# Veason-silverbullet/DIGAT

Measured on NVIDIA B200. Metric: impressions_scored_per_sec, higher is better.
Workload: dtype f32

## Files before the change

digat_b200/csrc/pair_attention_sparse.cuh:

```cuda
#pragma once
#include "common.cuh"
#include "tma.cuh"
#include "pair_attention.cuh"

namespace digat {

#ifndef DIGAT_SPARSE_WARPS
#define DIGAT_SPARSE_WARPS 10
#endif
#ifndef DIGAT_SPARSE_BUFS
#define DIGAT_SPARSE_BUFS 4
#endif
#ifndef DIGAT_SPARSE_MINCTAS
#define DIGAT_SPARSE_MINCTAS 2
#endif
#ifndef DIGAT_SPARSE_UNROLL
#define DIGAT_SPARSE_UNROLL 4
#endif
constexpr int kSparseConsumers = 32 * DIGAT_SPARSE_WARPS;
constexpr int kSparseThreads = kSparseConsumers + 32;
constexpr int kSparseBufs = DIGAT_SPARSE_BUFS;
constexpr int kSparseDc1 = 32, kSparseDc3 = 64;
constexpr int kSparseUnroll = DIGAT_SPARSE_UNROLL;

struct SparseGeom {
    int nch1, nch3;
    int G;
    int stagger_lo, stagger_hi;
    int tile_floats;
    int unit_floats;
    size_t smem;
};

__device__ __forceinline__ void consumer_sync() {
    asm volatile("bar.sync 1, %0;" :: "n"(kSparseConsumers) : "memory");
}

template <bool kIndexed, bool kMulti, bool kTrain = false>
__global__ void __launch_bounds__(kSparseThreads, DIGAT_SPARSE_MINCTAS)
graph_layer_fwd_sparse_kernel(const __grid_constant__ CUtensorMap map1, const __grid_constant__ CUtensorMap map3,
                              PairAttnArgs p, SparseGeom g) {
    extern __shared__ __align__(1024) uint8_t smem_raw[];
    const int tid = threadIdx.x, lane = tid & 31, warp = tid >> 5;
    const int n = p.n, D = p.D;
    const int b = kMulti ? blockIdx.x * g.G : blockIdx.x;
    const int N = kMulti ? min(g.G, p.B - b) * n : n;
    const int NB = kMulti ? g.G * n : n;
    const int src0 = kIndexed ? p.px_index[b] : b;

    float* ring = reinterpret_cast<float*>(smem_raw);
    uint64_t* full = reinterpret_cast<uint64_t*>(ring + kSparseBufs * g.unit_floats);
    uint64_t* empty = full + kSparseBufs;
    float* a_s = reinterpret_cast<float*>(empty + kSparseBufs);
    float* k3_s = a_s + D;
    float* score = k3_s + D;
    int* rowptr = reinterpret_cast<int*>(score + NB * n);
    uint16_t* meta = reinterpret_cast<uint16_t*>(rowptr + (NB + 2));
    uint8_t* adj_s = reinterpret_cast<uint8_t*>((reinterpret_cast<uintptr_t>(meta + NB * n) + 15) & ~(uintptr_t)15);
    uint8_t* uniform_row = adj_s + ((NB * n + 15) & ~15);
    uint8_t* dead_row = uniform_row + NB;
    int* pos_s = reinterpret_cast<int*>((reinterpret_cast<uintptr_t>(dead_row + NB) + 3) & ~(uintptr_t)3);
    int* n_act_s = pos_s + NB;
    uint8_t* act_list = reinterpret_cast<uint8_t*>(n_act_s + 1);

    if (tid == 0) {
        for (int i = 0; i < kSparseBufs; ++i) {
            mbar_init(&full[i], 1);
            mbar_init(&empty[i], kSparseConsumers / 32);
        }
        asm volatile("fence.mbarrier_init.release.cluster;" ::: "memory");
    }
#ifdef DIGAT_SPARSE_STAGGER
    if (blockIdx.x >= gridDim.y * 0 + (unsigned)g.stagger_lo && blockIdx.x < (unsigned)g.stagger_hi) __nanosleep(DIGAT_SPARSE_STAGGER);
#endif
    __syncthreads();
    const int n_loads = g.nch1 + g.nch3;

    if (warp == kSparseConsumers / 32) {
        if (lane == 0) {
            for (int l = 0; l < n_loads; ++l) {
                const int buf = l % kSparseBufs;
                float* dst = ring + buf * g.unit_floats;
                mbar_wait(&empty[buf], ((uint32_t)(l / kSparseBufs) & 1u) ^ 1u);
                if (l < g.nch1) {
                    mbar_arrive_expect_tx(&full[buf], 2u * NB * kSparseDc1 * 4u);
                    tma_load_2d(dst, &map1, &full[buf], D + l * kSparseDc1, src0 * n);
                    tma_load_2d(dst + g.tile_floats, &map1, &full[buf], 2 * D + l * kSparseDc1, src0 * n);
                } else {
                    mbar_arrive_expect_tx(&full[buf], (uint32_t)NB * kSparseDc3 * 4u);
                    tma_load_2d(dst, &map3, &full[buf], (l - g.nch1) * kSparseDc3, src0 * n);
                }
            }
        }
        return;
    }

#ifdef DIGAT_TC_TIMING
    const long long t0 = clock64();
    long long ta = t0, wait1 = 0, wait3 = 0;
#endif
    const float* __restrict__ gat_s = p.gat_s;
    for (int i = tid; i < D / 4; i += kSparseConsumers) {
        if (gat_s == nullptr) reinterpret_cast<float4*>(a_s)[i] = reinterpret_cast<const float4*>(p.a)[i];
        if (kIndexed) reinterpret_cast<float4*>(k3_s)[i] = reinterpret_cast<const float4*>(p.k3 + (size_t)b * p.ldk3)[i];
    }
    const bool have_csr = !kMulti && p.csr_rowptr != nullptr;
    if (have_csr) {
        const size_t cg = p.csr_index != nullptr ? (size_t)p.csr_index[b] : (size_t)b;
        const uint16_t* rp = p.csr_rowptr + cg * (n + 1);
        for (int i = tid; i <= n; i += kSparseConsumers) {
            const uint32_t raw = rp[i];
            rowptr[i] = (int)(raw & 0x7fffu);
            if (i > 0) uniform_row[i - 1] = (uint8_t)(raw >> 15);
        }
        if (p.Yc != nullptr)
            for (int i = tid; i < N; i += kSparseConsumers) pos_s[i] = p.row_pos[(size_t)b * n + i];
        consumer_sync();
        const int Ec = rowptr[n];
        const uint16_t* mg = p.csr_meta + cg * (size_t)n * n;
        for (int e = tid; e < Ec; e += kSparseConsumers) {
            const uint32_t mt = mg[e];
            meta[e] = (uint16_t)mt;
            score[e] = gat_s == nullptr ? 0.f
                                        : gat_s[((size_t)b * n + (mt & 255u)) * 2] + gat_s[((size_t)b * n + (mt >> 8)) * 2 + 1];
        }
        for (int i = tid; i < N; i += kSparseConsumers) dead_row[i] = rowptr[i + 1] == rowptr[i];
        if (warp == 0) {
            int run_a = 0;
            for (int base = 0; base < N; base += 32) {
                const int i = base + lane;
                const bool alive = i < N && rowptr[i + 1] != rowptr[i];
                const unsigned m = __ballot_sync(0xffffffffu, alive);
                if (alive) act_list[run_a + __popc(m & ((1u << lane) - 1u))] = (uint8_t)i;
                run_a += __popc(m);
            }
            if (lane == 0) *n_act_s = run_a;
        }
    } else {
    {
        const uint8_t* adj_g = p.adj + (p.adj_index != nullptr ? (size_t)p.adj_index[b] : (size_t)b) * n * n;
        const int n2 = N * n;
        if (((n2 | (int)(reinterpret_cast<uintptr_t>(adj_g) & 15)) & 15) == 0) {
            for (int i = tid; i < n2 / 16; i += kSparseConsumers)
                reinterpret_cast<uint4*>(adj_s)[i] = __ldg(reinterpret_cast<const uint4*>(adj_g) + i);
        } else {
            for (int i = tid; i < n2; i += kSparseConsumers) adj_s[i] = adj_g[i];
        }
        for (int i = tid; i < N; i += kSparseConsumers) {
            dead_row[i] = (p.row_active != nullptr && p.row_active[(size_t)b * n + i] == 0) ? 1 : 0;
            if (p.Yc != nullptr) pos_s[i] = p.row_pos[(size_t)b * n + i];
        }
    }
    consumer_sync();
#ifdef DIGAT_TC_TIMING
    ta = clock64();
#endif
    for (int i = warp; i < N; i += kSparseConsumers / 32) {
        const bool dead = dead_row[i] != 0;
        int deg = 0;
        if (!dead)
            for (int k = 0; k < (n + 31) / 32; ++k) {
                const int j = lane + 32 * k;
                deg += __popc(__ballot_sync(0xffffffffu, j < n && adj_s[i * n + j] != 0));
            }
        if (lane == 0) {
            uniform_row[i] = deg == 0 && !dead;
            rowptr[i + 1] = dead ? 0 : (deg == 0 ? n : deg);
        }
    }
    consumer_sync();
    if (warp == 0) {
        int run_e = 0;
        for (int base = 0; base < N; base += 32) {
            const int i = base + lane;
            int ve = i < N ? rowptr[i + 1] : 0;
#pragma unroll
            for (int o = 1; o < 32; o <<= 1) {
                const int te = __shfl_up_sync(0xffffffffu, ve, o);
                if (lane >= o) ve += te;
            }
            if (i < N) rowptr[i + 1] = run_e + ve;
            run_e += __shfl_sync(0xffffffffu, ve, 31);
        }
        if (lane == 0) rowptr[0] = 0;
        int run_a = 0;
        for (int base = 0; base < N; base += 32) {
            const int i = base + lane;
            const bool alive = i < N && dead_row[i] == 0;
            const unsigned m = __ballot_sync(0xffffffffu, alive);
            if (alive) act_list[run_a + __popc(m & ((1u << lane) - 1u))] = (uint8_t)i;
            run_a += __popc(m);
        }
        if (lane == 0) *n_act_s = run_a;
    }
    consumer_sync();
    for (int i = warp; i < N; i += kSparseConsumers / 32) {
        const int e0 = rowptr[i];
        const bool uni = uniform_row[i] != 0;
        if (dead_row[i] != 0) continue;
        const int node0 = kMulti ? (i / n) * n : 0;
        int filled = 0;
        for (int k = 0; k < (n + 31) / 32; ++k) {
            const int j = lane + 32 * k;
            const bool on = j < n && (uni || adj_s[i * n + j] != 0);
            const unsigned m = __ballot_sync(0xffffffffu, on);
            if (on) {
                const int e = e0 + filled + __popc(m & ((1u << lane) - 1u));
                meta[e] = (uint16_t)((node0 + j) | (i << 8));
                score[e] = gat_s == nullptr ? 0.f
                                            : gat_s[((size_t)b * n + node0 + j) * 2] + gat_s[((size_t)b * n + i) * 2 + 1];
            }
            filled += __popc(m);
        }
    }
    }
    const int E = rowptr[N];
    consumer_sync();

#ifdef DIGAT_TC_TIMING
    const long long t1 = clock64();
#endif
    const uint32_t a_off = (uint32_t)(reinterpret_cast<uint8_t*>(a_s) - smem_raw);
    const uint32_t k3_off = (uint32_t)(reinterpret_cast<uint8_t*>(k3_s) - smem_raw);
    for (int l = 0; l < g.nch1; ++l) {
        const int buf = l % kSparseBufs;
        const int c0 = l * kSparseDc1;
        const int wq = min(kSparseDc1, D - c0) >> 2;
        const uint32_t uoff = (uint32_t)(buf * g.unit_floats) * 4u;
        const uint32_t koff = uoff + (uint32_t)g.tile_floats * 4u;
        const uint32_t aoff = a_off + (uint32_t)c0 * 4u, k3off = k3_off + (uint32_t)c0 * 4u;
#ifdef DIGAT_TC_TIMING
        const long long tw0 = clock64();
#endif
        mbar_wait(&full[buf], (uint32_t)(l / kSparseBufs) & 1u);
#ifdef DIGAT_TC_TIMING
        wait1 += clock64() - tw0;
#endif
        for (int eb = warp * 32; eb < E; eb += 2 * kSparseConsumers) {
            const int e = eb + lane, e2 = e + kSparseConsumers;
            const bool one = e < E, two = e2 < E;
            const uint32_t mt = meta[one ? e : 0], mt2 = meta[two ? e2 : 0];
            const uint32_t uo = uoff + (mt & 255u) * (uint32_t)(kSparseDc1 * 4), ko = koff + (mt >> 8) * (uint32_t)(kSparseDc1 * 4);
            const uint32_t uo2 = uoff + (mt2 & 255u) * (uint32_t)(kSparseDc1 * 4), ko2 = koff + (mt2 >> 8) * (uint32_t)(kSparseDc1 * 4);
            const uint32_t ukey = ((uo >> 7) & 7u) << 4, kkey = ((ko >> 7) & 7u) << 4;
            const uint32_t ukey2 = ((uo2 >> 7) & 7u) << 4, kkey2 = ((ko2 >> 7) & 7u) << 4;
            uint64_t acc0 = 0ull, acc1 = 0ull, bcc0 = 0ull, bcc1 = 0ull;
            if (!__any_sync(0xffffffffu, two)) {
#pragma unroll kSparseUnroll
                for (int q = 0; q < wq; ++q) {
                    const uint32_t qo = (uint32_t)q * 16u;
                    const float4 av = *reinterpret_cast<const float4*>(smem_raw + aoff + qo);
                    const float4 k2 = *reinterpret_cast<const float4*>(smem_raw + ko + (qo ^ kkey));
                    const float4 u = *reinterpret_cast<const float4*>(smem_raw + uo + (qo ^ ukey));
                    uint64_t u01 = pack2(u.x, u.y), u23 = pack2(u.z, u.w);
                    if (kIndexed) {
                        const float4 kk = *reinterpret_cast<const float4*>(smem_raw + k3off + qo);
                        u01 = add2(pack2(kk.x, kk.y), u01);
                        u23 = add2(pack2(kk.z, kk.w), u23);
                    }
                    float s0, s1, s2, s3;
                    unpack2(add2(u01, pack2(k2.x, k2.y)), s0, s1);
                    unpack2(add2(u23, pack2(k2.z, k2.w)), s2, s3);
                    acc0 = fma2(pack2(av.x, av.y), pack2(fmaxf(s0, 0.f), fmaxf(s1, 0.f)), acc0);
                    acc1 = fma2(pack2(av.z, av.w), pack2(fmaxf(s2, 0.f), fmaxf(s3, 0.f)), acc1);
                }
            } else {
#pragma unroll kSparseUnroll
                for (int q = 0; q < wq; ++q) {
                    const uint32_t qo = (uint32_t)q * 16u;
                    const float4 av = *reinterpret_cast<const float4*>(smem_raw + aoff + qo);
                    const float4 k2 = *reinterpret_cast<const float4*>(smem_raw + ko + (qo ^ kkey));
                    const float4 u = *reinterpret_cast<const float4*>(smem_raw + uo + (qo ^ ukey));
                    const float4 k2b = *reinterpret_cast<const float4*>(smem_raw + ko2 + (qo ^ kkey2));
                    const float4 ub = *reinterpret_cast<const float4*>(smem_raw + uo2 + (qo ^ ukey2));
                    uint64_t u01 = pack2(u.x, u.y), u23 = pack2(u.z, u.w);
                    uint64_t v01 = pack2(ub.x, ub.y), v23 = pack2(ub.z, ub.w);
                    if (kIndexed) {
                        const float4 kk = *reinterpret_cast<const float4*>(smem_raw + k3off + qo);
                        const uint64_t k01 = pack2(kk.x, kk.y), k23 = pack2(kk.z, kk.w);
                        u01 = add2(k01, u01);
                        u23 = add2(k23, u23);
                        v01 = add2(k01, v01);
                        v23 = add2(k23, v23);
                    }
                    const uint64_t a01 = pack2(av.x, av.y), a23 = pack2(av.z, av.w);
                    float s0, s1, s2, s3;
                    unpack2(add2(u01, pack2(k2.x, k2.y)), s0, s1);
                    unpack2(add2(u23, pack2(k2.z, k2.w)), s2, s3);
                    acc0 = fma2(a01, pack2(fmaxf(s0, 0.f), fmaxf(s1, 0.f)), acc0);
                    acc1 = fma2(a23, pack2(fmaxf(s2, 0.f), fmaxf(s3, 0.f)), acc1);
                    unpack2(add2(v01, pack2(k2b.x, k2b.y)), s0, s1);
                    unpack2(add2(v23, pack2(k2b.z, k2b.w)), s2, s3);
                    bcc0 = fma2(a01, pack2(fmaxf(s0, 0.f), fmaxf(s1, 0.f)), bcc0);
                    bcc1 = fma2(a23, pack2(fmaxf(s2, 0.f), fmaxf(s3, 0.f)), bcc1);
                }
            }
            float a0, a1, b0, b1;
            unpack2(acc0, a0, a1);
            unpack2(acc1, b0, b1);
            if (one) score[e] += (a0 + a1) + (b0 + b1);
            if (two) {
                unpack2(bcc0, a0, a1);
                unpack2(bcc1, b0, b1);
                score[e2] += (a0 + a1) + (b0 + b1);
            }
        }
        __syncwarp();
        if (lane == 0) mbar_arrive(&empty[buf]);
    }
    consumer_sync();
#ifdef DIGAT_TC_TIMING
    const long long t2 = clock64();
#endif

    const bool train_out = kTrain && p.alpha_out != nullptr;
    float* __restrict__ e_alpha = train_out ? p.alpha_out + (size_t)b * n * n : nullptr;
    float* __restrict__ e_score = (train_out && p.score_out != nullptr) ? p.score_out + (size_t)b * n * n : nullptr;
    const uint8_t* __restrict__ keep_g = (kTrain && p.drop_keep != nullptr) ? p.drop_keep + (size_t)b * n * n : nullptr;
    auto finish_edge = [&](int e, float s_raw, float al) {
        if (e_score != nullptr) e_score[e] = s_raw;
        if (e_alpha != nullptr) e_alpha[e] = al;
        if (keep_g != nullptr) {
            const uint32_t mt = meta[e];
            al = keep_g[(mt >> 8) * n + (mt & 255u)] != 0 ? al * p.drop_scale : 0.f;
        }
        score[e] = al;
    };
    for (int i = warp; i < N; i += kSparseConsumers / 32) {
        const int e0 = rowptr[i], deg = rowptr[i + 1] - e0;
        if (deg == 0) continue;
        const bool uni = uniform_row[i] != 0;
        if (deg <= 32) {
            float m = -INFINITY, s = 0.f;
            if (lane < deg) {
                s = score[e0 + lane];
                m = uni ? kNegFill : (s > 0.f ? s : s * kLeakySlope);
            }
            const float mx1 = warp_max(m);
            const float ex = lane < deg ? expf(m - mx1) : 0.f;
            const float sum1 = warp_sum(ex);
            if (lane < deg) finish_edge(e0 + lane, s, ex / sum1);
            continue;
        }
        float v[kPairMaxNodes / 32], sr[kPairMaxNodes / 32];
        float mx = -INFINITY;
#pragma unroll
        for (int k = 0; k < kPairMaxNodes / 32; ++k) {
            const int t = lane + 32 * k;
            float m = -INFINITY;
            sr[k] = 0.f;
            if (t < deg) {
                const float s = score[e0 + t];
                sr[k] = s;
                m = uni ? kNegFill : (s > 0.f ? s : s * kLeakySlope);
            }
            v[k] = m;
            mx = fmaxf(mx, m);
        }
        mx = warp_max(mx);
        float sum = 0.f;
#pragma unroll
        for (int k = 0; k < kPairMaxNodes / 32; ++k) {
            const int t = lane + 32 * k;
            v[k] = (t < deg) ? expf(v[k] - mx) : 0.f;
            sum += v[k];
        }
        sum = warp_sum(sum);
#pragma unroll
        for (int k = 0; k < kPairMaxNodes / 32; ++k) {
            const int t = lane + 32 * k;
            if (t < deg) finish_edge(e0 + t, sr[k], v[k] / sum);
        }
    }
    consumer_sync();

#ifdef DIGAT_TC_TIMING
    const long long t3 = clock64();
#endif
    const int half_lane = lane & 15, sub = lane >> 4;
    constexpr int kXSlots = 2;
    constexpr int kRowPairStep = kSparseConsumers / 32;
    const int n_act = *n_act_s;
    auto row_of = [&](int slot) {
        const int k = 2 * (warp + slot * kRowPairStep) + sub;
        return k < n_act ? (int)act_list[k] : -1;
    };
    auto load_x = [&](int unit, int slot) {
        const int c0_ = unit * kSparseDc3;
        const int i_ = row_of(slot);
        return (unit < g.nch3 && i_ >= 0 && c0_ + 4 * half_lane < D)
                   ? ldg_stream(reinterpret_cast<const float4*>(p.X + ((size_t)src0 * n + i_) * D + c0_ + 4 * half_lane))
                   : make_float4(0.f, 0.f, 0.f, 0.f);
    };
    float4 xqa[kXSlots], xqb[kXSlots];
#pragma unroll
    for (int sl = 0; sl < kXSlots; ++sl) {
        xqa[sl] = load_x(0, sl);
        xqb[sl] = load_x(1, sl);
    }
    for (int l = g.nch1; l < n_loads; l += 2) {
        const bool pair = l + 1 < n_loads;
        const int bufa = l % kSparseBufs, bufb = (l + 1) % kSparseBufs;
        const int unit = l - g.nch1;
        const int c0 = unit * kSparseDc3;
        const int wqa = min(kSparseDc3, D - c0) >> 2;
        const int wqb = pair ? (min(kSparseDc3, D - c0 - kSparseDc3) >> 2) : 0;
        const float* Ha = ring + bufa * g.unit_floats + 4 * half_lane;
        const float* Hb = ring + bufb * g.unit_floats + 4 * half_lane;
        float4 xa[kXSlots], xb[kXSlots];
#pragma unroll
        for (int sl = 0; sl < kXSlots; ++sl) {
            xa[sl] = xqa[sl];
            xb[sl] = xqb[sl];
            xqa[sl] = load_x(unit + 2, sl);
            xqb[sl] = load_x(unit + 3, sl);
        }
#ifdef DIGAT_TC_TIMING
        const long long tw0 = clock64();
#endif
        mbar_wait(&full[bufa], (uint32_t)(l / kSparseBufs) & 1u);
        if (pair) mbar_wait(&full[bufb], (uint32_t)((l + 1) / kSparseBufs) & 1u);
#ifdef DIGAT_TC_TIMING
        wait3 += clock64() - tw0;
#endif
        const bool on_a = half_lane < wqa, on_b = half_lane < wqb;
        constexpr int kMaxPasses = (kPairMaxNodes / 2 + kRowPairStep - 1) / kRowPairStep;
#pragma unroll
        for (int sl = 0; sl < kMaxPasses; ++sl) {
            const int rp = warp + sl * kRowPairStep;
            if (2 * rp >= n_act) break;
            const int i = row_of(sl);
            if (i >= 0 && on_a) {
                const size_t xoff = ((size_t)src0 * n + i) * D + c0 + 4 * half_lane;
                const size_t yoff = ((size_t)b * n + i) * D + c0 + 4 * half_lane;
                float4 x0, x1 = make_float4(0.f, 0.f, 0.f, 0.f);
                if (sl < kXSlots) {
                    x0 = xa[sl < kXSlots ? sl : 0];
                    x1 = xb[sl < kXSlots ? sl : 0];
                } else {
                    x0 = ldg_stream(reinterpret_cast<const float4*>(p.X + xoff));
                    if (on_b) x1 = ldg_stream(reinterpret_cast<const float4*>(p.X + xoff + kSparseDc3));
                }
                uint64_t o01 = 0ull, o23 = 0ull, p01 = 0ull, p23 = 0ull;
                const int e1 = rowptr[i + 1];
                int e = rowptr[i];
                for (; e + 2 <= e1; e += 2) {
                    const float al0 = score[e], al1 = score[e + 1];
                    const uint32_t j0 = (meta[e] & 255u) * kSparseDc3, j1 = (meta[e + 1] & 255u) * kSparseDc3;
                    const float4 h0 = *reinterpret_cast<const float4*>(Ha + j0);
                    const float4 h1 = *reinterpret_cast<const float4*>(Ha + j1);
                    const float4 k0 = *reinterpret_cast<const float4*>(Hb + j0);
                    const float4 k1 = *reinterpret_cast<const float4*>(Hb + j1);
                    const uint64_t a0 = pack2(al0, al0), a1 = pack2(al1, al1);
                    o01 = fma2(a0, pack2(h0.x, h0.y), o01);
                    o23 = fma2(a0, pack2(h0.z, h0.w), o23);
                    p01 = fma2(a0, pack2(k0.x, k0.y), p01);
                    p23 = fma2(a0, pack2(k0.z, k0.w), p23);
                    o01 = fma2(a1, pack2(h1.x, h1.y), o01);
                    o23 = fma2(a1, pack2(h1.z, h1.w), o23);
                    p01 = fma2(a1, pack2(k1.x, k1.y), p01);
                    p23 = fma2(a1, pack2(k1.z, k1.w), p23);
                }
                if (e < e1) {
                    const float al = score[e];
                    const uint32_t j0 = (meta[e] & 255u) * kSparseDc3;
                    const float4 h = *reinterpret_cast<const float4*>(Ha + j0);
                    const float4 k = *reinterpret_cast<const float4*>(Hb + j0);
                    const uint64_t aa = pack2(al, al);
                    o01 = fma2(aa, pack2(h.x, h.y), o01);
                    o23 = fma2(aa, pack2(h.z, h.w), o23);
                    p01 = fma2(aa, pack2(k.x, k.y), p01);
                    p23 = fma2(aa, pack2(k.z, k.w), p23);
                }
                float4 y;
                unpack2(o01, y.x, y.y);
                unpack2(o23, y.z, y.w);
                if (kTrain && p.relu_mask_out != nullptr)
                    *reinterpret_cast<uchar4*>(p.relu_mask_out + yoff) = make_uchar4(y.x > 0.f, y.y > 0.f, y.z > 0.f, y.w > 0.f);
                y.x = fmaxf(y.x, 0.f) + x0.x;
                y.y = fmaxf(y.y, 0.f) + x0.y;
                y.z = fmaxf(y.z, 0.f) + x0.z;
                y.w = fmaxf(y.w, 0.f) + x0.w;
                stg_stream(reinterpret_cast<float4*>(p.Y + yoff), y);
                float* yc = p.Yc != nullptr ? p.Yc + (size_t)pos_s[i] * D + c0 + 4 * half_lane : nullptr;
                if (yc != nullptr) *reinterpret_cast<float4*>(yc) = y;
                if (on_b) {
                    unpack2(p01, y.x, y.y);
                    unpack2(p23, y.z, y.w);
                    if (kTrain && p.relu_mask_out != nullptr)
                        *reinterpret_cast<uchar4*>(p.relu_mask_out + yoff + kSparseDc3) = make_uchar4(y.x > 0.f, y.y > 0.f, y.z > 0.f, y.w > 0.f);
                    y.x = fmaxf(y.x, 0.f) + x1.x;
                    y.y = fmaxf(y.y, 0.f) + x1.y;
                    y.z = fmaxf(y.z, 0.f) + x1.z;
                    y.w = fmaxf(y.w, 0.f) + x1.w;
                    stg_stream(reinterpret_cast<float4*>(p.Y + yoff + kSparseDc3), y);
                    if (yc != nullptr) *reinterpret_cast<float4*>(yc + kSparseDc3) = y;
                }
            }
        }
        __syncwarp();
        if (lane == 0) {
            mbar_arrive(&empty[bufa]);
            if (pair) mbar_arrive(&empty[bufb]);
        }
    }
#ifdef DIGAT_TC_TIMING
    if (tid == 0 && (b % 1000) == 7)
        printf("graph %d E=%d n_act=%d csr=%d: setup %lld (loads %lld), phase1 %lld (waiting on TMA %lld), softmax %lld, phase3 %lld (waiting %lld)\n",
               b, E, n_act, (int)have_csr, t1 - t0, ta - t0, t2 - t1, wait1, t3 - t2, clock64() - t3, wait3);
#endif
}

inline void sparse_geometry(int n, int D, int G, SparseGeom* g) {
    const int NB = G * n;
    g->G = G;
    g->nch1 = (D + kSparseDc1 - 1) / kSparseDc1;
    g->nch3 = (D + kSparseDc3 - 1) / kSparseDc3;
    g->tile_floats = ((NB * kSparseDc1 * 4 + 1023) / 1024) * 1024 / 4;
    g->unit_floats = 2 * g->tile_floats;
    g->smem = (size_t)kSparseBufs * g->unit_floats * 4 + (size_t)2 * kSparseBufs * 8 + (size_t)2 * D * 4 +
              (size_t)NB * n * 4 + (size_t)(NB + 2) * 4 + (size_t)2 * NB * n + (size_t)((NB * n + 15) & ~15) + (size_t)2 * NB + (size_t)4 * NB + (size_t)NB + 8 + 64;
}

size_t graph_layer_fwd_sparse_smem(int n, int D) {
    SparseGeom g;
    sparse_geometry(n, D, 1, &g);
    return g.smem;
}

inline int sparse_graphs_per_cta(int n, int D, int B, int sm_count, size_t max_smem) {
    const size_t budget = (size_t)(227 * 1024) / DIGAT_SPARSE_MINCTAS - 1024 < max_smem ? (size_t)(227 * 1024) / DIGAT_SPARSE_MINCTAS - 1024 : max_smem;
    int best = 1;
    long best_cost = -1;
    for (int G = 1; G * n <= kPairMaxNodes && G <= B; ++G) {
        SparseGeom g;
        sparse_geometry(n, D, G, &g);
        if (G > 1 && g.smem > budget) break;
        const long ctas = (B + G - 1) / G, slots = (long)sm_count * DIGAT_SPARSE_MINCTAS;
        const long cost = ((ctas + slots - 1) / slots) * (G * (long)n + 24);
        if (best_cost < 0 || cost < best_cost) { best_cost = cost; best = G; }
    }
    return best;
}

int launch_graph_layer_fwd_sparse(const PairAttnArgs& args, int n_src, cudaStream_t st) {
    const DeviceInfo* di = device_info();
    if (!di) return fail(DIGAT_E_CUDA, "digat_graph_layer_fwd: no CUDA device");
    const bool indexed = args.px_index != nullptr;
    const bool training = args.alpha_out != nullptr || args.drop_keep != nullptr || args.relu_mask_out != nullptr;
    const int G = (indexed || args.adj_index != nullptr || training) ? 1
                  : sparse_graphs_per_cta(args.n, args.D, args.B, di->sm_count, (size_t)di->max_smem_optin);
    SparseGeom g;
    sparse_geometry(args.n, args.D, G, &g);
    g.stagger_lo = di->sm_count;
    g.stagger_hi = 2 * di->sm_count;
    DIGAT_REQUIRE(g.smem <= (size_t)di->max_smem_optin, "digat_graph_layer_fwd(sparse): needs %zu B shared memory", g.smem);
    CUtensorMap map1, map3;
    int rc;
    const int64_t src_graphs = indexed ? n_src : args.B;
    const int p_cols = args.gat_s != nullptr ? args.D : 3 * args.D;
    if (args.gat_s != nullptr) g.nch1 = 0;
    if ((rc = make_tensor_map_2d(&map1, args.P, src_graphs * args.n, p_cols, args.ldp, G * args.n, kSparseDc1, CU_TENSOR_MAP_SWIZZLE_128B)) != DIGAT_OK) return rc;
    if ((rc = make_tensor_map_2d(&map3, args.P, src_graphs * args.n, p_cols, args.ldp, G * args.n, kSparseDc3, CU_TENSOR_MAP_SWIZZLE_NONE)) != DIGAT_OK) return rc;
    const int grid = (args.B + G - 1) / G;
    if (indexed) {
        if (int rc_ = ensure_dynamic_smem(graph_layer_fwd_sparse_kernel<true, false>, (size_t)(g.smem))) return rc_;
        graph_layer_fwd_sparse_kernel<true, false><<<grid, kSparseThreads, g.smem, st>>>(map1, map3, args, g);
    } else if (training) {
        if (int rc_ = ensure_dynamic_smem(graph_layer_fwd_sparse_kernel<false, false, true>, (size_t)(g.smem))) return rc_;
        graph_layer_fwd_sparse_kernel<false, false, true><<<grid, kSparseThreads, g.smem, st>>>(map1, map3, args, g);
    } else if (G == 1) {
        if (int rc_ = ensure_dynamic_smem(graph_layer_fwd_sparse_kernel<false, false>, (size_t)(g.smem))) return rc_;
        graph_layer_fwd_sparse_kernel<false, false><<<grid, kSparseThreads, g.smem, st>>>(map1, map3, args, g);
    } else {
        if (int rc_ = ensure_dynamic_smem(graph_layer_fwd_sparse_kernel<false, true>, (size_t)(g.smem))) return rc_;
        graph_layer_fwd_sparse_kernel<false, true><<<grid, kSparseThreads, g.smem, st>>>(map1, map3, args, g);
    }
    return check_launch("digat_graph_layer_fwd(sparse)");
}

inline int launch_gat_layer_fwd(const float* Hm, int ldh, const float* s12, const uint8_t* adj, const float* X, float* Y,
                                int B, int n, int D, cudaStream_t st) {
    if (B == 0) return DIGAT_OK;
    DIGAT_REQUIRE(Hm && s12 && adj && X && Y, "digat_gat_layer_fwd: null pointer");
    DIGAT_REQUIRE(B >= 0 && n >= 1 && n <= kPairMaxNodes, "digat_gat_layer_fwd: n=%d outside [1,%d]", n, kPairMaxNodes);
    DIGAT_REQUIRE(D >= 4 && (D & 3) == 0 && D <= 1024, "digat_gat_layer_fwd: D=%d must be a multiple of 4 in [4,1024]", D);
    DIGAT_REQUIRE((ldh & 3) == 0 && ldh >= D, "digat_gat_layer_fwd: ldh=%d must be a multiple of 4 and >= D", ldh);
    DIGAT_REQUIRE(aligned16(Hm) && aligned16(X) && aligned16(Y), "digat_gat_layer_fwd: pointers must be 16-byte aligned");
    const DeviceInfo* di = device_info();
    if (!di) return fail(DIGAT_E_CUDA, "digat_gat_layer_fwd: no CUDA device");
    DIGAT_REQUIRE(graph_layer_fwd_sparse_smem(n, D) <= (size_t)di->max_smem_optin,
                  "digat_gat_layer_fwd: a graph of %d nodes x %d features does not fit one CTA", n, D);
    PairAttnArgs args{Hm, ldh, nullptr, adj, X, Y, B, n, D, nullptr, 1.f, nullptr, nullptr, nullptr,
                      nullptr, nullptr, nullptr, 0, nullptr, nullptr, nullptr};
    args.gat_s = s12;
    return launch_graph_layer_fwd_sparse(args, B, st);
}

inline int launch_gat_layer_train_fwd(const float* Hm, int ldh, const float* s12, const uint8_t* adj, const float* X, float* Y,
                                      int B, int n, int D, const uint8_t* drop_keep, float drop_scale, float* edge_score,
                                      float* edge_alpha, uint8_t* relu_mask, const uint16_t* csr_rowptr, const uint16_t* csr_meta,
                                      cudaStream_t st) {
    if (B == 0) return DIGAT_OK;
    DIGAT_REQUIRE(Hm && s12 && adj && X && Y && edge_score && edge_alpha && relu_mask && csr_rowptr && csr_meta,
                  "digat_gat_layer_train_fwd: null pointer");
    DIGAT_REQUIRE(B >= 0 && n >= 1 && n <= kPairMaxNodes, "digat_gat_layer_train_fwd: n=%d outside [1,%d]", n, kPairMaxNodes);
    DIGAT_REQUIRE(D >= 4 && (D & 3) == 0 && D <= 1024, "digat_gat_layer_train_fwd: D=%d must be a multiple of 4 in [4,1024]", D);
    DIGAT_REQUIRE((ldh & 3) == 0 && ldh >= D, "digat_gat_layer_train_fwd: ldh=%d must be a multiple of 4 and >= D", ldh);
    DIGAT_REQUIRE(aligned16(Hm) && aligned16(X) && aligned16(Y), "digat_gat_layer_train_fwd: pointers must be 16-byte aligned");
    const DeviceInfo* di = device_info();
    if (!di) return fail(DIGAT_E_CUDA, "digat_gat_layer_train_fwd: no CUDA device");
    DIGAT_REQUIRE(graph_layer_fwd_sparse_smem(n, D) <= (size_t)di->max_smem_optin,
                  "digat_gat_layer_train_fwd: a graph of %d nodes x %d features does not fit one CTA", n, D);
    PairAttnArgs args{Hm, ldh, nullptr, adj, X, Y, B, n, D, drop_keep, drop_scale, edge_score, edge_alpha, relu_mask,
                      nullptr, nullptr, nullptr, 0, nullptr, nullptr, nullptr};
    args.gat_s = s12;
    args.csr_rowptr = csr_rowptr;
    args.csr_meta = csr_meta;
    return launch_graph_layer_fwd_sparse(args, B, st);
}

}
```

Baseline: 751,000.

## Add grouped layer-0 sparse kernel sharing TMA-loaded source tiles across impressions

Adds a new kernel for the indexed (gathered) layer path that processes up to four consecutive batch entries pointing to the same source graph and CSR record in one pass. Each TMA-loaded P tile and the CSR metadata are reused across the group, with a per-impression k3 vector and score buffer. This cuts redundant tile loads and per-graph setup, at the cost of more registers per thread, a pass-size template dispatch, and fewer CTAs in the grid. The group size is limited by an edge-density heuristic.

```diff
diff --git a/digat_b200/csrc/pair_attention_sparse.cuh b/digat_b200/csrc/pair_attention_sparse.cuh
--- a/digat_b200/csrc/pair_attention_sparse.cuh
+++ b/digat_b200/csrc/pair_attention_sparse.cuh
@@ -1,4 +1,5 @@
 #pragma once
+#include <type_traits>
 #include "common.cuh"
 #include "tma.cuh"
 #include "pair_attention.cuh"
@@ -511,6 +512,321 @@
 #endif
 }
 
+#ifndef DIGAT_LAYER0_GROUP
+#define DIGAT_LAYER0_GROUP 4
+#endif
+constexpr int kLayer0Group = DIGAT_LAYER0_GROUP;
+
+template <int kMax, typename F>
+__device__ __forceinline__ void with_pass_size(int Q, F&& f) {
+    if constexpr (kMax > 1) {
+        if (Q < kMax) {
+            with_pass_size<kMax - 1>(Q, f);
+            return;
+        }
+    }
+    f(std::integral_constant<int, kMax>{});
+}
+
+template <int kGroup>
+__device__ __forceinline__ int grouped_pass_size(const PairAttnArgs& p, int k, int end) {
+    const int src = p.px_index[k];
+    const int cg = p.csr_index != nullptr ? p.csr_index[k] : k;
+    const int E = (int)(p.csr_rowptr[(size_t)cg * (p.n + 1) + p.n] & 0x7fffu);
+    const int qmax = E > 0 ? max(1, min(kGroup, p.n * p.n / E)) : kGroup;
+    int Q = 1;
+    while (Q < qmax && k + Q < end && p.px_index[k + Q] == src && (p.csr_index != nullptr ? p.csr_index[k + Q] : k + Q) == cg) ++Q;
+    return Q;
+}
+
+struct GroupedSmem {
+    uint32_t bars, a, k3, score, rowptr, pos, n_act, meta, uniform, act;
+    size_t bytes;
+};
+
+__host__ __device__ inline GroupedSmem grouped_smem_layout(int n, int D, int kGroup, int unit_floats) {
+    GroupedSmem s;
+    uint32_t o = (uint32_t)kSparseBufs * unit_floats * 4;
+    s.bars = o;     o += 2 * kSparseBufs * 8;
+    s.a = o;        o += D * 4;
+    s.k3 = o;       o += kGroup * D * 4;
+    s.score = o;    o += n * n * 4;
+    s.rowptr = o;   o += (n + 2) * 4;
+    s.pos = o;      o += kGroup * n * 4;
+    s.n_act = o;    o += 4;
+    s.meta = o;     o += n * n * 2;
+    s.uniform = o;  o += n;
+    s.act = o;      o += n;
+    s.bytes = o + 16;
+    return s;
+}
+
+template <int kGroup>
+__global__ void __launch_bounds__(kSparseThreads, DIGAT_SPARSE_MINCTAS)
+graph_layer_fwd_grouped_kernel(const __grid_constant__ CUtensorMap map1, const __grid_constant__ CUtensorMap map3,
+                               PairAttnArgs p, SparseGeom g) {
+    extern __shared__ __align__(1024) uint8_t smem_raw[];
+    const int tid = threadIdx.x, lane = tid & 31, warp = tid >> 5;
+    const int n = p.n, D = p.D;
+    const int begin = blockIdx.x * kGroup, end = min(p.B, begin + kGroup);
+    const GroupedSmem sl = grouped_smem_layout(n, D, kGroup, g.unit_floats);
+    float* ring = reinterpret_cast<float*>(smem_raw);
+    uint64_t* full = reinterpret_cast<uint64_t*>(smem_raw + sl.bars);
+    uint64_t* empty = full + kSparseBufs;
+    float* a_s = reinterpret_cast<float*>(smem_raw + sl.a);
+    float* k3_s = reinterpret_cast<float*>(smem_raw + sl.k3);
+    float* score = reinterpret_cast<float*>(smem_raw + sl.score);
+    int* rowptr = reinterpret_cast<int*>(smem_raw + sl.rowptr);
+    int* pos_s = reinterpret_cast<int*>(smem_raw + sl.pos);
+    int* n_act_s = reinterpret_cast<int*>(smem_raw + sl.n_act);
+    uint16_t* meta = reinterpret_cast<uint16_t*>(smem_raw + sl.meta);
+    uint8_t* uniform_row = smem_raw + sl.uniform;
+    uint8_t* act_list = smem_raw + sl.act;
+
+    if (tid == 0) {
+        for (int i = 0; i < kSparseBufs; ++i) {
+            mbar_init(&full[i], 1);
+            mbar_init(&empty[i], kSparseConsumers / 32);
+        }
+        asm volatile("fence.mbarrier_init.release.cluster;" ::: "memory");
+    }
+    __syncthreads();
+    const int n_loads = g.nch1 + g.nch3;
+
+    if (warp == kSparseConsumers / 32) {
+        if (lane == 0) {
+            int L = 0;
+            for (int k = begin; k < end;) {
+                const int Q = grouped_pass_size<kGroup>(p, k, end);
+                const int src0 = p.px_index[k];
+                for (int l = 0; l < n_loads; ++l, ++L) {
+                    const int buf = L % kSparseBufs;
+                    float* dst = ring + buf * g.unit_floats;
+                    mbar_wait(&empty[buf], ((uint32_t)(L / kSparseBufs) & 1u) ^ 1u);
+                    if (l < g.nch1) {
+                        mbar_arrive_expect_tx(&full[buf], 2u * n * kSparseDc1 * 4u);
+                        tma_load_2d(dst, &map1, &full[buf], D + l * kSparseDc1, src0 * n);
+                        tma_load_2d(dst + g.tile_floats, &map1, &full[buf], 2 * D + l * kSparseDc1, src0 * n);
+                    } else {
+                        mbar_arrive_expect_tx(&full[buf], (uint32_t)n * kSparseDc3 * 4u);
+                        tma_load_2d(dst, &map3, &full[buf], (l - g.nch1) * kSparseDc3, src0 * n);
+                    }
+                }
+                k += Q;
+            }
+        }
+        return;
+    }
+
+    for (int i = tid; i < D / 4; i += kSparseConsumers) reinterpret_cast<float4*>(a_s)[i] = reinterpret_cast<const float4*>(p.a)[i];
+    const int half_lane = lane & 15, sub = lane >> 4;
+    int L = 0, cg_prev = -1;
+    for (int k = begin; k < end;) {
+        const int Q = grouped_pass_size<kGroup>(p, k, end);
+        const int src0 = p.px_index[k];
+        const int cg = p.csr_index != nullptr ? p.csr_index[k] : k;
+        const bool new_record = cg != cg_prev;
+        cg_prev = cg;
+        consumer_sync();
+        const uint16_t* rp = p.csr_rowptr + (size_t)cg * (n + 1);
+        if (new_record)
+            for (int i = tid; i <= n; i += kSparseConsumers) {
+                const uint32_t raw = rp[i];
+                rowptr[i] = (int)(raw & 0x7fffu);
+                if (i > 0) uniform_row[i - 1] = (uint8_t)(raw >> 15);
+            }
+        for (int i = tid; i < Q * (D / 4); i += kSparseConsumers) {
+            const int gq = i / (D / 4), c = i - gq * (D / 4);
+            reinterpret_cast<float4*>(k3_s + gq * D)[c] = reinterpret_cast<const float4*>(p.k3 + (size_t)(k + gq) * p.ldk3)[c];
+        }
+        if (p.Yc != nullptr)
+            for (int i = tid; i < Q * n; i += kSparseConsumers) pos_s[i] = p.row_pos[(size_t)k * n + i];
+        consumer_sync();
+        const int E = rowptr[n];
+        if (new_record) {
+            const uint16_t* mg = p.csr_meta + (size_t)cg * n * n;
+            for (int e = tid; e < E; e += kSparseConsumers) meta[e] = mg[e];
+            if (warp == 0) {
+                int run_a = 0;
+                for (int base = 0; base < n; base += 32) {
+                    const int i = base + lane;
+                    const bool alive = i < n && rowptr[i + 1] != rowptr[i];
+                    const unsigned m = __ballot_sync(0xffffffffu, alive);
+                    if (alive) act_list[run_a + __popc(m & ((1u << lane) - 1u))] = (uint8_t)i;
+                    run_a += __popc(m);
+                }
+                if (lane == 0) *n_act_s = run_a;
+            }
+        }
+        for (int e = tid; e < Q * E; e += kSparseConsumers) score[e] = 0.f;
+        consumer_sync();
+        const int n_act = *n_act_s;
+
+        with_pass_size<kGroup>(Q, [&](auto qc) {
+            constexpr int kQ = decltype(qc)::value;
+            for (int l = 0; l < g.nch1; ++l, ++L) {
+                const int buf = L % kSparseBufs;
+                const int c0 = l * kSparseDc1;
+                const int wq = min(kSparseDc1, D - c0) >> 2;
+                const uint32_t uoff = (uint32_t)(buf * g.unit_floats) * 4u;
+                const uint32_t koff = uoff + (uint32_t)g.tile_floats * 4u;
+                const uint32_t aoff = sl.a + (uint32_t)c0 * 4u, k3off = sl.k3 + (uint32_t)c0 * 4u;
+                mbar_wait(&full[buf], (uint32_t)(L / kSparseBufs) & 1u);
+                for (int eb = warp * 32; eb < E; eb += kSparseConsumers) {
+                    const int e = eb + lane;
+                    const bool one = e < E;
+                    const uint32_t mt = meta[one ? e : 0];
+                    const uint32_t uo = uoff + (mt & 255u) * (uint32_t)(kSparseDc1 * 4), ko = koff + (mt >> 8) * (uint32_t)(kSparseDc1 * 4);
+                    const uint32_t ukey = ((uo >> 7) & 7u) << 4, kkey = ((ko >> 7) & 7u) << 4;
+                    uint64_t acc[kQ][2];
+#pragma unroll
+                    for (int gq = 0; gq < kQ; ++gq) acc[gq][0] = acc[gq][1] = 0ull;
+#pragma unroll kSparseUnroll
+                    for (int q = 0; q < wq; ++q) {
+                        const uint32_t qo = (uint32_t)q * 16u;
+                        const float4 av = *reinterpret_cast<const float4*>(smem_raw + aoff + qo);
+                        const float4 k2 = *reinterpret_cast<const float4*>(smem_raw + ko + (qo ^ kkey));
+                        const float4 k1 = *reinterpret_cast<const float4*>(smem_raw + uo + (qo ^ ukey));
+                        const uint64_t a01 = pack2(av.x, av.y), a23 = pack2(av.z, av.w);
+                        const uint64_t k201 = pack2(k2.x, k2.y), k223 = pack2(k2.z, k2.w);
+                        const uint64_t k101 = pack2(k1.x, k1.y), k123 = pack2(k1.z, k1.w);
+#pragma unroll
+                        for (int gq = 0; gq < kQ; ++gq) {
+                            const float4 kk = *reinterpret_cast<const float4*>(smem_raw + k3off + (uint32_t)(gq * D) * 4u + qo);
+                            float s0, s1, s2, s3;
+                            unpack2(add2(add2(pack2(kk.x, kk.y), k101), k201), s0, s1);
+                            unpack2(add2(add2(pack2(kk.z, kk.w), k123), k223), s2, s3);
+                            acc[gq][0] = fma2(a01, pack2(fmaxf(s0, 0.f), fmaxf(s1, 0.f)), acc[gq][0]);
+                            acc[gq][1] = fma2(a23, pack2(fmaxf(s2, 0.f), fmaxf(s3, 0.f)), acc[gq][1]);
+                        }
+                    }
+                    if (one) {
+#pragma unroll
+                        for (int gq = 0; gq < kQ; ++gq) {
+                            float a0, a1, b0, b1;
+                            unpack2(acc[gq][0], a0, a1);
+                            unpack2(acc[gq][1], b0, b1);
+                            score[gq * E + e] += (a0 + a1) + (b0 + b1);
+                        }
+                    }
+                }
+                __syncwarp();
+                if (lane == 0) mbar_arrive(&empty[buf]);
+            }
+            consumer_sync();
+
+            for (int r = warp; r < kQ * n_act; r += kSparseConsumers / 32) {
+                const int gq = r / n_act;
+                const int i = act_list[r - gq * n_act];
+                float* sc = score + gq * E;
+                const int e0 = rowptr[i], deg = rowptr[i + 1] - e0;
+                const bool uni = uniform_row[i] != 0;
+                if (deg <= 32) {
+                    float m = -INFINITY;
+                    if (lane < deg) {
+                        const float s = sc[e0 + lane];
+                        m = uni ? kNegFill : (s > 0.f ? s : s * kLeakySlope);
+                    }
+                    const float mx1 = warp_max(m);
+                    const float ex = lane < deg ? expf(m - mx1) : 0.f;
+                    const float sum1 = warp_sum(ex);
+                    if (lane < deg) sc[e0 + lane] = ex / sum1;
+                    continue;
+                }
+                float v[kPairMaxNodes / 32];
+                float mx = -INFINITY;
+#pragma unroll
+                for (int kk = 0; kk < kPairMaxNodes / 32; ++kk) {
+                    const int t = lane + 32 * kk;
+                    float m = -INFINITY;
+                    if (t < deg) {
+                        const float s = sc[e0 + t];
+                        m = uni ? kNegFill : (s > 0.f ? s : s * kLeakySlope);
+                    }
+                    v[kk] = m;
+                    mx = fmaxf(mx, m);
+                }
+                mx = warp_max(mx);
+                float sum = 0.f;
+#pragma unroll
+                for (int kk = 0; kk < kPairMaxNodes / 32; ++kk) {
+                    const int t = lane + 32 * kk;
+                    v[kk] = (t < deg) ? expf(v[kk] - mx) : 0.f;
+                    sum += v[kk];
+                }
+                sum = warp_sum(sum);
+#pragma unroll
+                for (int kk = 0; kk < kPairMaxNodes / 32; ++kk) {
+                    const int t = lane + 32 * kk;
+                    if (t < deg) sc[e0 + t] = v[kk] / sum;
+                }
+            }
+            consumer_sync();
+
+            for (int u = 0; u < g.nch3; ++u, ++L) {
+                const int buf = L % kSparseBufs;
+                const int c0 = u * kSparseDc3;
+                const int wq = min(kSparseDc3, D - c0) >> 2;
+                const float* H = ring + buf * g.unit_floats + 4 * half_lane;
+                mbar_wait(&full[buf], (uint32_t)(L / kSparseBufs) & 1u);
+                if (half_lane < wq) {
+                    for (int r = 2 * warp + sub; r < n_act; r += kSparseConsumers / 16) {
+                        const int i = act_list[r];
+                        const float4 x = ldg_stream(reinterpret_cast<const float4*>(p.X + ((size_t)src0 * n + i) * D + c0 + 4 * half_lane));
+                        uint64_t o[kQ][2];
+#pragma unroll
+                        for (int gq = 0; gq < kQ; ++gq) o[gq][0] = o[gq][1] = 0ull;
+                        const int e1 = rowptr[i + 1];
+                        int e = rowptr[i];
+                        for (; e + 2 <= e1; e += 2) {
+                            const float4 h0 = *reinterpret_cast<const float4*>(H + (meta[e] & 255u) * kSparseDc3);
+                            const float4 h1 = *reinterpret_cast<const float4*>(H + (meta[e + 1] & 255u) * kSparseDc3);
+                            const uint64_t h001 = pack2(h0.x, h0.y), h023 = pack2(h0.z, h0.w);
+                            const uint64_t h101 = pack2(h1.x, h1.y), h123 = pack2(h1.z, h1.w);
+#pragma unroll
+                            for (int gq = 0; gq < kQ; ++gq) {
+                                const float al0 = score[gq * E + e], al1 = score[gq * E + e + 1];
+                                const uint64_t a0 = pack2(al0, al0), a1 = pack2(al1, al1);
+                                o[gq][0] = fma2(a0, h001, o[gq][0]);
+                                o[gq][1] = fma2(a0, h023, o[gq][1]);
+                                o[gq][0] = fma2(a1, h101, o[gq][0]);
+                                o[gq][1] = fma2(a1, h123, o[gq][1]);
+                            }
+                        }
+                        if (e < e1) {
+                            const float4 h = *reinterpret_cast<const float4*>(H + (meta[e] & 255u) * kSparseDc3);
+                            const uint64_t h01 = pack2(h.x, h.y), h23 = pack2(h.z, h.w);
+#pragma unroll
+                            for (int gq = 0; gq < kQ; ++gq) {
+                                const float al = score[gq * E + e];
+                                const uint64_t aa = pack2(al, al);
+                                o[gq][0] = fma2(aa, h01, o[gq][0]);
+                                o[gq][1] = fma2(aa, h23, o[gq][1]);
+                            }
+                        }
+#pragma unroll
+                        for (int gq = 0; gq < kQ; ++gq) {
+                            float4 y;
+                            unpack2(o[gq][0], y.x, y.y);
+                            unpack2(o[gq][1], y.z, y.w);
+                            y.x = fmaxf(y.x, 0.f) + x.x;
+                            y.y = fmaxf(y.y, 0.f) + x.y;
+                            y.z = fmaxf(y.z, 0.f) + x.z;
+                            y.w = fmaxf(y.w, 0.f) + x.w;
+                            stg_stream(reinterpret_cast<float4*>(p.Y + ((size_t)(k + gq) * n + i) * D + c0 + 4 * half_lane), y);
+                            if (p.Yc != nullptr)
+                                *reinterpret_cast<float4*>(p.Yc + (size_t)pos_s[gq * n + i] * D + c0 + 4 * half_lane) = y;
+                        }
+                    }
+                }
+                __syncwarp();
+                if (lane == 0) mbar_arrive(&empty[buf]);
+            }
+        });
+        k += Q;
+    }
+}
+
 inline void sparse_geometry(int n, int D, int G, SparseGeom* g) {
     const int NB = G * n;
     g->G = G;
@@ -563,7 +879,13 @@
     if ((rc = make_tensor_map_2d(&map1, args.P, src_graphs * args.n, p_cols, args.ldp, G * args.n, kSparseDc1, CU_TENSOR_MAP_SWIZZLE_128B)) != DIGAT_OK) return rc;
     if ((rc = make_tensor_map_2d(&map3, args.P, src_graphs * args.n, p_cols, args.ldp, G * args.n, kSparseDc3, CU_TENSOR_MAP_SWIZZLE_NONE)) != DIGAT_OK) return rc;
     const int grid = (args.B + G - 1) / G;
-    if (indexed) {
+    if (indexed && args.csr_rowptr != nullptr && !training && g_layer_mode != 3) {
+        const size_t smem = grouped_smem_layout(args.n, args.D, kLayer0Group, g.unit_floats).bytes;
+        DIGAT_REQUIRE(smem <= (size_t)di->max_smem_optin, "digat_graph_layer_fwd(grouped): needs %zu B shared memory", smem);
+        if (int rc_ = ensure_dynamic_smem(graph_layer_fwd_grouped_kernel<kLayer0Group>, smem)) return rc_;
+        graph_layer_fwd_grouped_kernel<kLayer0Group><<<(args.B + kLayer0Group - 1) / kLayer0Group, kSparseThreads, smem, st>>>(
+            map1, map3, args, g);
+    } else if (indexed) {
         if (int rc_ = ensure_dynamic_smem(graph_layer_fwd_sparse_kernel<true, false>, (size_t)(g.smem))) return rc_;
         graph_layer_fwd_sparse_kernel<true, false><<<grid, kSparseThreads, g.smem, st>>>(map1, map3, args, g);
     } else if (training) {
```

After: 782,900, median of 6. 4.2% higher.
